# ur-whitelab/hoomd-tf

Measured on AMD Instinct MI355X. Metric: MD steps/sec + achieved HBM GB/s, 131072 particles NN=128 (131k-particle box of the BASELINE metric), higher is better.
Workload: dtype f32

## Files before the change

### hoomd_tf_amd/_lib.py

```python
import ctypes as C
import os

import torch

_HERE = os.path.dirname(os.path.abspath(__file__))
LIB_PATH = os.environ.get("HTF_AMD_LIB") or os.path.join(_HERE, "libhtf_amd.so")

HTF_OK, HTF_ERR_INVALID, HTF_ERR_DEVICE, HTF_ERR_NLIST_OVERFLOW, HTF_ERR_SKEWED_BOX, HTF_ERR_NOMEM = range(6)
HTF_F32, HTF_F64 = 0, 1
HTF_TF2HOOMD, HTF_HOOMD2TF = 0, 1
POT_NONE, POT_LJ, POT_WCA, POT_RINV_POLY, POT_SIMPLE, POT_PAIR_MLP, POT_GAUSS, POT_LJ_PARAM, POT_TOPK_MLP, POT_JIT = range(10)
JIT_READS_OWN_TYPE = 1
OPT_SGD, OPT_ADAM, OPT_NADAM = range(3)
OPT_STATE_FLOATS = 24
ACT_LINEAR, ACT_TANH = 0, 1
MLP_FP32, MLP_BF16, MLP_SPLIT, MLP_SPLIT16 = 0, 1, 2, 3
MAX_POLY_TERMS = 8


class NlistOverflowError(RuntimeError):
    """'Neighbor list is full!' -- tf.errors.InvalidArgumentError upstream
    (simmodel.py:220-224, test_tensorflow.py:830-848)."""


# ... 36 lines not shown
MBOX_MAX_MSG, MBOX_MAX_RANKS, IPC_HANDLE_BYTES = 8, 64, 64


class Mailbox(C.Structure):
    _fields_ = [("remote", C.c_void_p * MBOX_MAX_MSG), ("remote_signal", C.c_void_p * MBOX_MAX_MSG), ("mine", C.c_void_p),
                ("my_signal", C.c_void_p), ("state", C.c_void_p), ("spin_limit", C.c_uint), ("half_units", C.c_uint)]


class ReduceBox(C.Structure):
    _fields_ = [("remote", C.c_void_p * MBOX_MAX_RANKS), ("mine", C.c_void_p), ("state", C.c_void_p), ("spin_limit", C.c_uint),
                ("world", C.c_int), ("rank", C.c_int)]


class Mirror(C.Structure):
    _fields_ = [("src", C.c_void_p * MIRROR_MAX), ("dst", C.c_void_p * MIRROR_MAX), ("words", C.c_uint * MIRROR_MAX), ("n", C.c_uint)]


class Nlist(C.Structure):
    _fields_ = [("box", Box), ("r_list", C.c_double), ("ncell3", C.c_int * 3), ("stencil3", C.c_int * 3), ("pitch", C.c_uint),
                ("type_split", C.c_int)] + [(name, C.c_void_p) for name in (
                    "cell_of", "scratch", "cell_start", "order", "pos_sorted", "ranges", "n_neigh", "head_list", "nlist", "max_neigh",
                    "ref", "counter")] + [("image_L", C.c_double * 3)]


class BrickWork(C.Structure):
    _fields_ = [("key", C.c_void_p), ("order", C.c_void_p), ("sort_scratch", C.c_void_p), ("start1", C.c_void_p),
                ("start2", C.c_void_p), ("tmp_pos", C.c_void_p), ("tmp_vel", C.c_void_p)]


class PotentialDesc(C.Structure):
# ... 279 lines not shown
```

### hoomd_tf_amd/csrc/standin.hip

```cpp
#include <cstdlib>

#include "htf_common.h"
#include "box_math.h"
#include "htf_standin.h"
#include "standin_gate.h"
#include "key_sort.h"

namespace htf {

template <typename T>
__global__ __launch_bounds__(256) void nve_step_kernel(typename Vec4<T>::type *__restrict__ pos,
                                                       typename Vec4<T>::type *__restrict__ vel,
                                                       const typename Vec4<T>::type *__restrict__ force,
                                                       unsigned N, T dt, SBox<T> b) {
    unsigned i = blockIdx.x * blockDim.x + threadIdx.x;
    if (i >= N) return;
    auto p = pos[i];
    auto v = vel[i];
    nve_advance<T>(p, v, force[i], dt, b);
    pos[i] = p;
    vel[i] = v;
}

template <typename T>
__global__ __launch_bounds__(1024) void max_disp_kernel(const typename Vec4<T>::type *__restrict__ pos,
                                                        const typename Vec4<T>::type *__restrict__ ref, unsigned N,
                                                        SBox<T> b, float *__restrict__ out) {
    __shared__ float s_max[16];
    unsigned i = blockIdx.x * blockDim.x + threadIdx.x;
    float d2 = 0.f;
    if (i < N) {
        auto p = pos[i];
        auto r = ref[i];
        T dx = mimg<T>(p.x - r.x, b.L[0], b.Linv[0], b.periodic[0]);
        T dy = mimg<T>(p.y - r.y, b.L[1], b.Linv[1], b.periodic[1]);
        T dz = mimg<T>(p.z - r.z, b.L[2], b.Linv[2], b.periodic[2]);
        d2 = (float)(dx * dx + dy * dy + dz * dz);
        if (!(d2 == d2)) d2 = 0.f;
    }
    for (int m = 1; m < 64; m <<= 1) d2 = fmaxf(d2, __shfl_xor(d2, m));
    if ((threadIdx.x & 63) == 0) s_max[threadIdx.x >> 6] = d2;
    __syncthreads();
    if (threadIdx.x < 16) {
        d2 = s_max[threadIdx.x];
        for (int m = 1; m < 16; m <<= 1) d2 = fmaxf(d2, __shfl_xor(d2, m));
        if (threadIdx.x == 0 && __float_as_uint(d2) > *(volatile unsigned *)out)
            atomicMax((unsigned *)out, __float_as_uint(d2));
    }
}

template <typename T>
__global__ __launch_bounds__(1024) void check_disp_kernel(const typename Vec4<T>::type *__restrict__ pos,
                                                          const typename Vec4<T>::type *__restrict__ ref, unsigned N,
                                                          SBox<T> b, unsigned *__restrict__ work, float *__restrict__ out,
                                                          float *__restrict__ h_out, htfs_mirror mirror) {
    __shared__ float s_max[16];
    __shared__ unsigned s_last;
    unsigned i = blockIdx.x * blockDim.x + threadIdx.x;
    float d2 = 0.f;
    if (i < N) {
        auto p = pos[i];
        auto r = ref[i];
        T dx = mimg<T>(p.x - r.x, b.L[0], b.Linv[0], b.periodic[0]);
        T dy = mimg<T>(p.y - r.y, b.L[1], b.Linv[1], b.periodic[1]);
        T dz = mimg<T>(p.z - r.z, b.L[2], b.Linv[2], b.periodic[2]);
        d2 = (float)(dx * dx + dy * dy + dz * dz);
        if (!(d2 == d2)) d2 = 0.f;
    }
    for (int m = 1; m < 64; m <<= 1) d2 = fmaxf(d2, __shfl_xor(d2, m));
    if ((threadIdx.x & 63) == 0) s_max[threadIdx.x >> 6] = d2;
    if (threadIdx.x == 0) s_last = 0u;
    __syncthreads();
    if (threadIdx.x < 16) {
        d2 = s_max[threadIdx.x];
        for (int m = 1; m < 16; m <<= 1) d2 = fmaxf(d2, __shfl_xor(d2, m));
        if (threadIdx.x == 0) {
            if (__float_as_uint(d2) > *(volatile unsigned *)work) atomicMax(work, __float_as_uint(d2));
            __threadfence();
            if (atomicAdd(work + 1, 1u) == gridDim.x - 1u) s_last = 1u;
        }
    }
    __syncthreads();
    if (s_last == 0u) return;
// ... 4 lines not shown
    }
    __threadfence_system();
    __syncthreads();
    if (threadIdx.x == 0) {
        const float worst = __uint_as_float(atomicExch(work, 0u));
        const unsigned cycle = __float_as_uint(out[1]) + 1u;
        out[0] = worst;
        out[1] = __uint_as_float(cycle);
        work[1] = 0u;
        if (h_out != nullptr) {
            h_out[0] = worst;
            __threadfence_system();
            *(volatile unsigned *)(h_out + 1) = cycle;
        }
    }
}

template <typename T>
__device__ __forceinline__ int cell_coord(T x, T lo, T Linv, int n) {
    int c = (int)floor((x - lo) * Linv * (T)n);
    return c < 0 ? 0 : (c >= n ? n - 1 : c);
}

template <typename T>
__global__ __launch_bounds__(256) void cell_index_kernel(const typename Vec4<T>::type *__restrict__ pos, unsigned Ntot,
                                                         SBox<T> b, int nx, int ny, int nz,
                                                         unsigned *__restrict__ cell_of, Gate gate) {
    if (gate.closed()) return;
    unsigned i = blockIdx.x * blockDim.x + threadIdx.x;
    if (i >= Ntot) return;
// ... 47 lines not shown
        o.x = cell_start[rowbase + a0];
        o.y = (cell_start[rowbase + a1 + 1] - o.x) | (wrap_y << kRangeWrapShift) | (wrap_z << (kRangeWrapShift + 2));
        if (b1 >= b0) {
            o.z = cell_start[rowbase + b0];
            o.w = (cell_start[rowbase + b1 + 1] - o.z) | ((b0 == 0 ? 2u : 1u) << kRangeWrapShift);
        }
    }
    table[t] = o;
}
__global__ __launch_bounds__(256) void cell_ranges_kernel(RangesArgs a, Gate gate) {
    if (gate.closed()) return;
    cell_ranges_body(blockIdx.x * blockDim.x + threadIdx.x, a);
}

template <typename T, int G, bool SHIFT>
__global__ __launch_bounds__(256) void build_nlist_kernel(const typename Vec4<T>::type *__restrict__ pos,
                                                          const typename Vec4<T>::type *__restrict__ pos_sorted,
                                                          unsigned N, SBox<T> b, T rl2, int nx, int ny, int nz,
                                                          int wx, int wy, int wz,
                                                          const unsigned *__restrict__ cell_start, unsigned pitch,
                                                          int type_split,
                                                          unsigned *__restrict__ n_neigh, unsigned *__restrict__ head_list,
                                                          unsigned *__restrict__ nlist, unsigned *__restrict__ max_neigh,
                                                          const uint4 *__restrict__ ranges, Gate gate) {
    if (gate.closed()) return;
    const unsigned lane = threadIdx.x & 63u, g = lane % G, sub = lane / G;
    const unsigned i = ((blockIdx.x * blockDim.x + threadIdx.x) >> 6) * (64 / G) + sub;
    const bool in_range = i < N;
    const auto pi = pos[in_range ? i : 0];
    const bool active = in_range && !is_inert(pi.x);
    const int cx = cell_coord<T>(pi.x, b.lo[0], b.Linv[0], nx);
    const int cy = cell_coord<T>(pi.y, b.lo[1], b.Linv[1], ny);
    const int cz = cell_coord<T>(pi.z, b.lo[2], b.Linv[2], nz);
    const bool side_i = type_split >= 0 && scalar_as_int(pi.w) >= type_split;
    unsigned count = 0;
    unsigned *row = nlist + (size_t)(active ? i : 0) * pitch;
    const int nrow = (2 * wy + 1) * (2 * wz + 1);
    const uint4 *mine = ranges + (size_t)((cz * ny + cy) * nx + cx) * nrow;
    uint4 rg_next = active ? mine[0] : make_uint4(0u, 0u, 0u, 0u);
    for (int r = 0; r < nrow; ++r) {
// ... 25 lines not shown
                unsigned long long hits = ballot64(m_idx < n) & ballot64(k != i) & ballot64(ddx * ddx + ddy * ddy + ddz * ddz <= rl2);
                if (type_split >= 0) {
                    asm volatile("" ::: "memory");
                    hits &= ballot64(((tag & kTagSide) != 0u) == side_i);
                }
                const unsigned seg = (unsigned)(hits >> (G * sub)) & (G >= 32 ? ~0u : ((1u << G) - 1u));
                const unsigned rank = count + (unsigned)__popc(seg & ((1u << g) - 1u));
                if (inverse_ballot64(hits) && rank < pitch) row[rank] = k;
                count += (unsigned)__popc(seg);
            }
        }
    }
    if (in_range && g == 0) {
        n_neigh[i] = count < pitch ? count : pitch;
        head_list[i] = i * pitch;
        if (count > *(volatile unsigned *)max_neigh) atomicMax(max_neigh, count);
    }
}


__device__ __forceinline__ void set_tag(float &w, unsigned tag) { w = __uint_as_float(tag); }
__device__ __forceinline__ void set_tag(double &w, unsigned tag) { w = __longlong_as_double((long long)tag); }
__device__ __forceinline__ float bcast_lane_t(float v, unsigned lane) {
    return __int_as_float(__builtin_amdgcn_readlane(__float_as_int(v), (int)lane));
}
__device__ __forceinline__ double bcast_lane_t(double v, unsigned lane) {
    const long long q = __double_as_longlong(v);
    const unsigned lo = (unsigned)__builtin_amdgcn_readlane((int)(unsigned)q, (int)lane);
    const unsigned hi = (unsigned)__builtin_amdgcn_readlane((int)(unsigned)(q >> 32), (int)lane);
    return __longlong_as_double((long long)(((unsigned long long)hi << 32) | lo));
}
__device__ __forceinline__ unsigned bperm_u(unsigned lane_idx, unsigned v) {
    return (unsigned)__builtin_amdgcn_ds_bpermute((int)(lane_idx << 2), (int)v);
}
__device__ __forceinline__ float bperm_t(unsigned lane_idx, float v) { return __uint_as_float(bperm_u(lane_idx, __float_as_uint(v))); }
__device__ __forceinline__ double bperm_t(unsigned lane_idx, double v) {
    const unsigned long long q = (unsigned long long)__double_as_longlong(v);
    const unsigned lo = bperm_u(lane_idx, (unsigned)q), hi = bperm_u(lane_idx, (unsigned)(q >> 32));
    return __longlong_as_double((long long)(((unsigned long long)hi << 32) | lo));
}
constexpr int kCellBatch = 8;

template <typename T, bool SHIFT>
__global__ __launch_bounds__(256) void build_nlist_cells_kernel(const typename Vec4<T>::type *__restrict__ pos_sorted, unsigned N,
                                                                SBox<T> b, T rl2, unsigned ncell, int nrow,
                                                                const unsigned *__restrict__ cell_start, unsigned pitch,
                                                                int type_split, unsigned *__restrict__ n_neigh,
                                                                unsigned *__restrict__ head_list, unsigned *__restrict__ nlist,
                                                                unsigned *__restrict__ max_neigh,
                                                                const uint4 *__restrict__ ranges, unsigned split, Gate gate) {
    if (gate.closed()) return;
    using V4 = typename Vec4<T>::type;
    const unsigned lane = threadIdx.x & 63u;
    const unsigned wv = __builtin_amdgcn_readfirstlane((blockIdx.x * blockDim.x + threadIdx.x) >> 6);
    const unsigned c = wv / split, b0 = wv % split;
    if (c >= ncell) return;
    const unsigned p_begin = cell_start[c], p_end = cell_start[c + 1];
    if (p_begin + b0 * (unsigned)kCellBatch >= p_end) return;
    if (p_end - p_begin <= 64u) {
        const bool local = lane < p_end - p_begin && ((unsigned)scalar_as_int(pos_sorted[p_begin + lane].w) & ~kTagSide) < N;
        if (ballot64(local) == 0ull) return;
    }

    unsigned beg = 0u, len = 0u;
    T shx = (T)0, shy = (T)0, shz = (T)0;
    if (lane < 2u * (unsigned)nrow) {
// ... 81 lines not shown
                    hits &= ballot64(((tag ^ tag_p[p]) & kTagSide) == 0u);
                }
                const unsigned rank = __builtin_amdgcn_mbcnt_hi((unsigned)(hits >> 32), __builtin_amdgcn_mbcnt_lo((unsigned)hits, count[p]));
                if (inverse_ballot64(hits) && rank < pitch) nlist[row_p[p] + rank] = k;
                count[p] += (unsigned)__builtin_popcountll(hits);
            }
        }
        unsigned cnt = 0u;
#pragma unroll
        for (int p = 0; p < kCellBatch; ++p) cnt = lane == (unsigned)p ? count[p] : cnt;
        if (lane < np) {
            const unsigned i = my_tag & ~kTagSide;
            if (i < N) {
                n_neigh[i] = cnt < pitch ? cnt : pitch;
                head_list[i] = i * pitch;
                if (cnt > *(volatile unsigned *)max_neigh) atomicMax(max_neigh, cnt);
            }
        }
    }
}

}

using namespace htf;

extern "C" int htfs_nve_step(void *d_pos, void *d_vel, const void *d_force, int dtype, unsigned N, double dt,
                             const htf_box *box, htf_stream stream) {
    HTF_REQUIRE(d_pos && d_vel && d_force && box, "htfs_nve_step: null pointer");
    if (N == 0) return HTF_OK;
    unsigned grid = (N + 255) / 256;
    if (dtype == HTF_F32)
        hipLaunchKernelGGL((nve_step_kernel<float>), dim3(grid), dim3(256), 0, (hipStream_t)stream, (float4 *)d_pos, (float4 *)d_vel, (const float4 *)d_force, N, (float)dt, make_sbox<float>(box));
    else
        hipLaunchKernelGGL((nve_step_kernel<double>), dim3(grid), dim3(256), 0, (hipStream_t)stream, (double4 *)d_pos, (double4 *)d_vel, (const double4 *)d_force, N, dt, make_sbox<double>(box));
// ... 30 lines not shown
        hipLaunchKernelGGL((check_disp_kernel<float>), dim3(grid), dim3(1024), 0, (hipStream_t)stream, (const float4 *)d_pos, (const float4 *)d_ref, N, make_sbox<float>(box), d_work, d_out, h_out, mr);
    else
        hipLaunchKernelGGL((check_disp_kernel<double>), dim3(grid), dim3(1024), 0, (hipStream_t)stream, (const double4 *)d_pos, (const double4 *)d_ref, N, make_sbox<double>(box), d_work, d_out, h_out, mr);
    return check_launch("check_disp_kernel");
}

namespace htf {
struct Reimage {
    double L[3], c[3];
};
template <typename T>
__device__ __forceinline__ T reimage1(T x, double L, double c) {
    return L > 0.0 ? (T)((double)x - L * rint(((double)x - c) / L)) : x;
}

template <typename V>
__global__ __launch_bounds__(256) void bins_finish_kernel(RangesArgs ra, unsigned nb_ranges, V *__restrict__ dest, const V *__restrict__ src,
                                                          const int *__restrict__ order, unsigned n, int type_split, V *__restrict__ ref,
                                                          unsigned n_ref, unsigned *__restrict__ counter, Reimage im, Gate gate) {
    if (gate.closed()) return;
    if (blockIdx.x < nb_ranges) {
        cell_ranges_body(blockIdx.x * blockDim.x + threadIdx.x, ra);
        return;
    }
    const unsigned i = (blockIdx.x - nb_ranges) * blockDim.x + threadIdx.x;
    if (i == 0 && counter != nullptr) *counter += 1u;
    if (i >= n || i >= ra.cell_start[ra.nx * ra.ny * ra.nz]) return;
    const unsigned k = (unsigned)order[i];
    V p = src[k];
    if (ref != nullptr && k < n_ref) ref[k] = p;
    p.x = reimage1(p.x, im.L[0], im.c[0]);
    p.y = reimage1(p.y, im.L[1], im.c[1]);
    p.z = reimage1(p.z, im.L[2], im.c[2]);
    set_tag(p.w, k | ((type_split >= 0 && scalar_as_int(p.w) >= type_split) ? kTagSide : 0u));
    dest[i] = p;
}

template <typename T>
__global__ __launch_bounds__(256) void cell_index_count_kernel(const typename Vec4<T>::type *__restrict__ pos, unsigned Ntot, SBox<T> b,
                                                               int nx, int ny, int nz, unsigned *__restrict__ cell_of,
                                                               unsigned *__restrict__ count, Reimage im, Gate gate) {
    if (gate.closed()) return;
    unsigned i = blockIdx.x * blockDim.x + threadIdx.x;
    if (i >= Ntot) return;
    auto p = pos[i];
    if (is_inert(p.x)) {
        cell_of[i] = kDeadCell;
        return;
    }
    int cx = cell_coord<T>(reimage1(p.x, im.L[0], im.c[0]), b.lo[0], b.Linv[0], nx);
// ... 78 lines not shown
}

__global__ __launch_bounds__(256) void cell_scatter_kernel(const unsigned *__restrict__ cell_of, unsigned n,
                                                           unsigned *__restrict__ cursor, unsigned *__restrict__ order, Gate gate) {
    if (gate.closed()) return;
    const unsigned i = blockIdx.x * blockDim.x + threadIdx.x;
    if (i < n && cell_of[i] != kDeadCell) order[atomicAdd(&cursor[cell_of[i]], 1u)] = i;
}

__global__ __launch_bounds__(256) void cell_order_kernel(const unsigned *__restrict__ start, unsigned ncell,
                                                         unsigned *__restrict__ order, unsigned *__restrict__ count, Gate gate) {
    if (gate.closed()) return;
    const unsigned c = blockIdx.x * blockDim.x + threadIdx.x;
    if (c >= ncell) return;
    count[c] = 0u;
    const unsigned b = start[c], e = start[c + 1];
    for (unsigned i = b + 1; i < e; ++i) {
        const unsigned v = order[i];
        unsigned j = i;
        while (j > b && order[j - 1] > v) {
            order[j] = order[j - 1];
            --j;
        }
        order[j] = v;
    }
}
}

static int zero_counts(unsigned *count, unsigned ncell, hipStream_t s) {
    HTF_REQUIRE(((uintptr_t)count & 15) == 0, "binning scratch must be 16-byte aligned (cell_scan_kernel reads it with 16-byte loads)");
    HTF_CHECK_HIP(hipMemsetAsync(count, 0, (size_t)ncell * sizeof(unsigned), s));
    return HTF_OK;
}

extern "C" int htfs_cell_sort(const unsigned *d_cell_of, unsigned Ntot, unsigned ncell, unsigned *d_scratch,
                              unsigned *d_cell_start, unsigned *d_order, htf_stream stream) {
    using namespace htf;
    HTF_REQUIRE(d_cell_of && d_scratch && d_cell_start && d_order, "htfs_cell_sort: null pointer");
    HTF_REQUIRE(ncell > 0, "htfs_cell_sort: no cells");
    hipStream_t s = (hipStream_t)stream;
// ... 120 lines not shown
}

extern "C" int htfs_cell_index(const void *d_pos, int dtype, unsigned Ntot, const htf_box *box, const int *ncell3,
                               unsigned *d_cell_of, htf_stream stream) {
    HTF_REQUIRE(d_pos && box && ncell3 && d_cell_of, "htfs_cell_index: null pointer");
    if (Ntot == 0) return HTF_OK;
    unsigned grid = (Ntot + 255) / 256;
    if (dtype == HTF_F32)
        hipLaunchKernelGGL((cell_index_kernel<float>), dim3(grid), dim3(256), 0, (hipStream_t)stream, (const float4 *)d_pos, Ntot, make_sbox<float>(box), ncell3[0], ncell3[1], ncell3[2], d_cell_of, kOpenGate);
    else
        hipLaunchKernelGGL((cell_index_kernel<double>), dim3(grid), dim3(256), 0, (hipStream_t)stream, (const double4 *)d_pos, Ntot, make_sbox<double>(box), ncell3[0], ncell3[1], ncell3[2], d_cell_of, kOpenGate);
    return check_launch("cell_index_kernel");
}

struct FinishArgs {
    unsigned n;
    htf::Reimage im;
};

static int build_nlist_impl(const htfs_nlist *l, const void *d_pos, int dtype, unsigned N, htf_stream stream, htf::Gate gate,
                            const FinishArgs *fin) {
    using namespace htf;
    HTF_REQUIRE(l && d_pos && l->pos_sorted && l->cell_start && l->n_neigh && l->head_list && l->nlist && l->max_neigh,
                "htfs_build_nlist: null pointer");
    const htf_box *box = &l->box;
    const int *ncell3 = l->ncell3, *stencil3 = l->stencil3;
    const unsigned *d_cell_start = l->cell_start;
    const void *d_pos_sorted = l->pos_sorted;
    const unsigned pitch = l->pitch;
    const int type_split = l->type_split;
    const double r_list = l->r_list;
    unsigned *d_n_neigh = l->n_neigh, *d_head_list = l->head_list, *d_nlist = l->nlist, *d_max_neigh = l->max_neigh;
    HTF_REQUIRE(pitch > 0, "htfs_build_nlist: pitch must be > 0");
    for (int d = 0; d < 3; ++d) {
        const double w = (box->hi[d] - box->lo[d]) / ncell3[d];
        const int sw = stencil3[d];
        HTF_REQUIRE((sw == 0 && ncell3[d] == 1) || (sw >= 1 && sw <= 2 && ncell3[d] >= 2 * sw + 1 && w * sw >= r_list * (1.0 - 1e-12)),
                    "htfs_build_nlist: along %d need 1 cell, or >= 2w+1 cells with w cells spanning r_list (got %d cells of %g, stencil %d, r_list %g)",
                    d, ncell3[d], w, sw, r_list);
    }
    if (N == 0) return HTF_OK;
    const unsigned ncell = (unsigned)(ncell3[0] * ncell3[1] * ncell3[2]);
    const unsigned nrow = (unsigned)((2 * stencil3[1] + 1) * (2 * stencil3[2] + 1));
    HTF_REQUIRE(l->ranges && ((uintptr_t)l->ranges & 15) == 0, "htfs_build_nlist: ranges must be a 16-byte aligned table of 4 * ncell * rows words");
    uint4 *d_ranges = (uint4 *)l->ranges;
    const RangesArgs ra = {ncell3[0], ncell3[1], ncell3[2], stencil3[0], stencil3[1], stencil3[2], (int)box->periodic[0],
                           (int)box->periodic[1], (int)box->periodic[2], d_cell_start, d_ranges, d_max_neigh};
    const unsigned nb_ranges = (ncell * nrow + 255) / 256;
    if (fin == nullptr) {
        hipLaunchKernelGGL(cell_ranges_kernel, dim3(nb_ranges), dim3(256), 0, (hipStream_t)stream, ra, gate);
    } else {
        const unsigned nb = nb_ranges + (fin->n + 255) / 256 + (fin->n == 0 ? 1u : 0u);
        if (dtype == HTF_F32)
            hipLaunchKernelGGL((bins_finish_kernel<float4>), dim3(nb), dim3(256), 0, (hipStream_t)stream, ra, nb_ranges, (float4 *)l->pos_sorted,
                               (const float4 *)d_pos, (const int *)l->order, fin->n, type_split, (float4 *)l->ref, N, l->counter, fin->im, gate);
        else
            hipLaunchKernelGGL((bins_finish_kernel<double4>), dim3(nb), dim3(256), 0, (hipStream_t)stream, ra, nb_ranges, (double4 *)l->pos_sorted,
                               (const double4 *)d_pos, (const int *)l->order, fin->n, type_split, (double4 *)l->ref, N, l->counter, fin->im, gate);
    }
    const bool fine = stencil3[0] == 2 || stencil3[1] == 2 || stencil3[2] == 2;
#define HTFS_NL(T, V4, G)                                                                                              \
    if (shift) HTFS_NL_(T, V4, G, true); else HTFS_NL_(T, V4, G, false)
#define HTFS_NL_(T, V4, G, S)                                                                                          \
    hipLaunchKernelGGL((build_nlist_kernel<T, G, S>), dim3((N + 4 * (64 / G) - 1) / (4 * (64 / G))), dim3(256), 0, (hipStream_t)stream, \
                       (const V4 *)d_pos, (const V4 *)d_pos_sorted, N, make_sbox<T>(box), (T)(r_list * r_list), ncell3[0],  \
                       ncell3[1], ncell3[2], stencil3[0], stencil3[1], stencil3[2], d_cell_start, pitch,      \
                       type_split, d_n_neigh, d_head_list, d_nlist, d_max_neigh, (const uint4 *)d_ranges, gate)
#define HTFS_NLC(T, V4)                                                                                                \
    if (shift) HTFS_NLC_(T, V4, true); else HTFS_NLC_(T, V4, false)
#define HTFS_NLC_(T, V4, S)                                                                                            \
    hipLaunchKernelGGL((build_nlist_cells_kernel<T, S>), dim3((ncell * cell_split + 3) / 4), dim3(256), 0, (hipStream_t)stream, \
                       (const V4 *)d_pos_sorted, N, make_sbox<T>(box), (T)(r_list * r_list), ncell, (int)nrow, d_cell_start, pitch, \
                       type_split, d_n_neigh, d_head_list, d_nlist, d_max_neigh, (const uint4 *)d_ranges, cell_split, gate)
    bool shift = true;
    for (int d = 0; d < 3; ++d) shift = shift && (!box->periodic[d] || ncell3[d] >= 7);
#ifdef HTF_AB_VARIANTS
    static const bool per_particle = std::getenv("HTFS_NLIST_PER_PARTICLE") != nullptr, per_cell = std::getenv("HTFS_NLIST_PER_CELL") != nullptr;
#else
    constexpr bool per_particle = false, per_cell = false;
#endif
    const bool reimaged = fin != nullptr && (fin->im.L[0] > 0.0 || fin->im.L[1] > 0.0 || fin->im.L[2] > 0.0);
    const bool by_cell = per_cell || reimaged || (!per_particle && ncell >= 1024u);
    const unsigned cell_split = ncell <= 12288u ? 2u : 1u;
    if (by_cell) {
        if (dtype == HTF_F32) { HTFS_NLC(float, float4); } else { HTFS_NLC(double, double4); }
    } else if (dtype == HTF_F32) {
        if (fine) { HTFS_NL(float, float4, 8); } else { HTFS_NL(float, float4, 16); }
    } else {
        if (fine) { HTFS_NL(double, double4, 8); } else { HTFS_NL(double, double4, 16); }
    }
#undef HTFS_NL
#undef HTFS_NL_
#undef HTFS_NLC
#undef HTFS_NLC_
    return check_launch("build_nlist_kernel");
}

extern "C" int htfs_build_nlist(const htfs_nlist *nl, const void *d_pos, int dtype, unsigned N, htf_stream stream) {
    return build_nlist_impl(nl, d_pos, dtype, N, stream, htf::kOpenGate, nullptr);
}

static int rebuild_nlist_impl(const htfs_nlist *l, const void *d_pos, int dtype, unsigned N, unsigned Ntot, bool scratch_clean,
                              htf_stream stream, htf::Gate gate) {
    using namespace htf;
    HTF_REQUIRE(l && d_pos && l->cell_of && l->scratch && l->cell_start && l->order && l->pos_sorted, "htfs_rebuild_nlist: null pointer");
    HTF_REQUIRE(Ntot >= N, "htfs_rebuild_nlist: Ntot %u < N %u", Ntot, N);
    if (N == 0) return HTF_OK;
    const htf_box *box = &l->box;
    const int *ncell3 = l->ncell3;
    const unsigned ncell = (unsigned)(ncell3[0] * ncell3[1] * ncell3[2]);
    HTF_REQUIRE(ncell > 0, "htfs_rebuild_nlist: no cells");
    hipStream_t s = (hipStream_t)stream;
    unsigned *count = l->scratch, *cursor = l->scratch + ncell;
    if (!scratch_clean)
        if (int rc = zero_counts(count, ncell, s)) return rc;
    const unsigned grid = (Ntot + 255) / 256;
    Reimage im = {};
    for (int d = 0; d < 3; ++d) {
        im.L[d] = !box->periodic[d] ? l->image_L[d] : 0.0;
        im.c[d] = 0.5 * (box->lo[d] + box->hi[d]);
        HTF_REQUIRE(im.L[d] == 0.0 || im.L[d] >= box->hi[d] - box->lo[d], "htfs_rebuild_nlist: image length %g along axis %d is shorter than the grid", im.L[d], d);
    }
    if (dtype == HTF_F32)
        hipLaunchKernelGGL((cell_index_count_kernel<float>), dim3(grid), dim3(256), 0, s, (const float4 *)d_pos, Ntot, make_sbox<float>(box),
                           ncell3[0], ncell3[1], ncell3[2], l->cell_of, count, im, gate);
    else
        hipLaunchKernelGGL((cell_index_count_kernel<double>), dim3(grid), dim3(256), 0, s, (const double4 *)d_pos, Ntot, make_sbox<double>(box),
                           ncell3[0], ncell3[1], ncell3[2], l->cell_of, count, im, gate);
    hipLaunchKernelGGL(cell_scan_kernel, dim3((ncell + kScanChunk - 1) / kScanChunk), dim3(kScanThreads), 0, s, count, ncell, l->cell_start, cursor, gate);
    hipLaunchKernelGGL(cell_scatter_kernel, dim3(grid), dim3(256), 0, s, l->cell_of, Ntot, cursor, l->order, gate);
    hipLaunchKernelGGL(cell_order_kernel, dim3((ncell + 255) / 256), dim3(256), 0, s, l->cell_start, ncell, l->order, count, gate);
    const FinishArgs fin = {Ntot, im};
    return build_nlist_impl(l, d_pos, dtype, N, stream, gate, &fin);
}

extern "C" int htfs_rebuild_nlist(const htfs_nlist *nl, const void *d_pos, int dtype, unsigned N, unsigned Ntot, int scratch_clean,
                                  htf_stream stream) {
    return rebuild_nlist_impl(nl, d_pos, dtype, N, Ntot, scratch_clean != 0, stream, htf::kOpenGate);
}

extern "C" int htfs_check_rebuild_nlist(const htfs_nlist *nl, const void *d_pos, int dtype, unsigned N, unsigned Ntot, int scratch_clean,
                                        float *d_disp2, double threshold2, unsigned *d_stat2, unsigned *h_stat2, htf_stream stream) {
    HTF_REQUIRE(nl && nl->ref && d_disp2 && d_stat2, "htfs_check_rebuild_nlist: null pointer");
    if (N == 0) return HTF_OK;
    HTF_CHECK_HIP(hipMemsetAsync(d_disp2, 0, sizeof(float), (hipStream_t)stream));
    int rc = htfs_max_displacement2(d_pos, nl->ref, dtype, N, &nl->box, d_disp2, stream);
    if (rc != HTF_OK) return rc;
    htfs_nlist l = *nl;
    l.max_neigh = d_stat2;
    l.counter = d_stat2 + 1;
    rc = rebuild_nlist_impl(&l, d_pos, dtype, N, Ntot, scratch_clean != 0, stream, htf::Gate{d_disp2, (float)threshold2});
    if (rc != HTF_OK) return rc;
    if (h_stat2 != nullptr)
        HTF_CHECK_HIP(hipMemcpyAsync(h_stat2, d_stat2, 2 * sizeof(unsigned), hipMemcpyDeviceToHost, (hipStream_t)stream));
    return HTF_OK;
}
```

### hoomd_tf_amd/standin.py

```python
import ctypes as C
import math
import os

import numpy as np
import torch

from . import _lib, ops
from ._lib import lib, check
from .ops import raw_stream


def fcc_positions(n_cells, rho):
    a = (4.0 / rho) ** (1.0 / 3.0)
    L = n_cells * a
    ijk = np.stack(np.meshgrid(*[np.arange(n_cells)] * 3, indexing="ij"), -1).reshape(-1, 3)
    base = np.array([[0.25, 0.25, 0.25], [0.75, 0.75, 0.25], [0.75, 0.25, 0.75], [0.25, 0.75, 0.75]])
    pos = ((ijk[:, None, :] + base[None]) * a).reshape(-1, 3) - L / 2
    return pos, np.array([L, L, L]), a


def sc_positions(n_cells, rho):
    a = (1.0 / rho) ** (1.0 / 3.0)
    L = n_cells * a
    ijk = np.stack(np.meshgrid(*[np.arange(n_cells)] * 3, indexing="ij"), -1).reshape(-1, 3)
# ... 97 lines not shown
        self.sys = system
        self.deferred_reference = bool(deferred_reference)
        self._rule = None
        self._dd_prev = None
        self._dd_i = 0
        self.device_decision = bool(device_decision)
        self.sort_particles = bool(sort_particles)
        self.r_cut = float(r_cut)
        self.r_buff = float(r_buff)
        self.check_period = int(check_period)
        self._desc = _lib.Nlist()
        self.pitch = pitch
        self.n_neigh = self.head_list = self.nlist = None
        self.type_split = -1
        self._ref = None
        self._disp = torch.zeros(1, dtype=torch.float32, device=system.device)
        self._max = torch.zeros(1, dtype=torch.int32, device=system.device)
        self._desc.max_neigh = self._max.data_ptr()
        self.n_builds = 0
        self._subscribers = []
        self.domain = None
        self._sbox_key = None
        self._scr_n = None
        self._grid = None
        self._scratch_clean = None
        self._step_done = None
        self._capturing = False
        self._stat = self._stat_host = self._stat_event = None
        self._max_host = self._max_event = None
        self._mirrored = False

# ... 758 lines not shown
```

### include/htf_standin.h

```cpp
#ifndef HTF_STANDIN_H_
#define HTF_STANDIN_H_
#include "htf_amd.h"
#ifdef __cplusplus
extern "C" {
#endif

HTF_API int htfs_nve_step(void *d_pos, void *d_vel, const void *d_force, int dtype, unsigned N,
                          double dt, const htf_box *box, htf_stream stream);

HTF_API int htfs_max_displacement2(const void *d_pos, const void *d_ref, int dtype, unsigned N,
                                   const htf_box *box, float *d_out, htf_stream stream);

#define HTFS_MIRROR_MAX 4
typedef struct htfs_mirror {
    const void *src[HTFS_MIRROR_MAX];
    void *dst[HTFS_MIRROR_MAX];
    unsigned words[HTFS_MIRROR_MAX];
    unsigned n;
} htfs_mirror;
HTF_API int htfs_check_displacement2(const void *d_pos, const void *d_ref, int dtype, unsigned N, const htf_box *box,
                                     unsigned *d_work, float *d_out, float *h_out, const htfs_mirror *mirror, htf_stream stream);

#define HTFS_RANGE_WORDS(ncell, stencil_y, stencil_z) (4u * (size_t)(ncell) * (2u * (stencil_y) + 1u) * (2u * (stencil_z) + 1u))
typedef struct htfs_nlist {
// ... 19 lines not shown
} htfs_nlist;

HTF_API int htfs_cell_index(const void *d_pos, int dtype, unsigned Ntot, const htf_box *box,
                            const int *ncell3, unsigned *d_cell_of, htf_stream stream);
HTF_API int htfs_cell_sort(const unsigned *d_cell_of, unsigned Ntot, unsigned ncell, unsigned *d_scratch,
                           unsigned *d_cell_start, unsigned *d_order, htf_stream stream);
HTF_API int htfs_gather4_tagged(void *d_dest, const void *d_src, const int *d_order, int dtype, unsigned n, int type_split,
                                htf_stream stream);
HTF_API int htfs_gather4_tagged_live(void *d_dest, const void *d_src, const int *d_order, int dtype, unsigned n_max,
                                     const unsigned *d_n_live, int type_split, htf_stream stream);
HTF_API int htfs_build_nlist(const htfs_nlist *nl, const void *d_pos, int dtype, unsigned N, htf_stream stream);

HTF_API int htfs_rebuild_nlist(const htfs_nlist *nl, const void *d_pos, int dtype, unsigned N, unsigned Ntot, int scratch_clean,
                               htf_stream stream);

HTF_API int htfs_check_rebuild_nlist(const htfs_nlist *nl, const void *d_pos, int dtype, unsigned N, unsigned Ntot, int scratch_clean,
                                     float *d_disp2, double threshold2, unsigned *d_stat2, unsigned *h_stat2, htf_stream stream);

HTF_API int htfs_slab_classify(const void *d_pos, int dtype, unsigned N, const void *d_bounds, int world, int rank,
                               double r_ghost, unsigned *d_key, htf_stream stream);

HTF_API int htfs_key_sort16(const unsigned *d_key, unsigned N, unsigned *d_scratch, unsigned *d_start, unsigned *d_order,
                            htf_stream stream);

#define HTFS_MAX_SEGMENTS 16
HTF_API int htfs_segment_copy(void *d_dst, const void *d_src, unsigned row_bytes, unsigned n_segments,
                              const unsigned *src_start, const unsigned *dst_start, const unsigned *count, htf_stream stream);

#define HTFS_BRICK_MAX_MSG 8
#define HTFS_BRICK_MAX_P 64
// ... 126 lines not shown
```

Before: 13410.

## Fuse displacement check and stat reporting into nlist rebuild kernels

Replaces the memset plus max-displacement launch with a single self-resetting check_gate kernel that publishes the max displacement via a ticket counter. The separate cell_order sort kernel is folded into bins_finish, which now runs per cell and sorts small cells in registers with an odd-even network. The host memcpy of the stat words is replaced by a last-workgroup tree ticket inside the nlist build kernel that writes the stats directly to host memory. Together these remove several launches and a copy per step, at the cost of extra atomics and a per-cell finish whose load balance depends on cell occupancy.

```diff
diff --git a/hoomd_tf_amd/_lib.py b/hoomd_tf_amd/_lib.py
--- a/hoomd_tf_amd/_lib.py
+++ b/hoomd_tf_amd/_lib.py
@@ -74,6 +74,9 @@
 
 class Mirror(C.Structure):
     _fields_ = [("src", C.c_void_p * MIRROR_MAX), ("dst", C.c_void_p * MIRROR_MAX), ("words", C.c_uint * MIRROR_MAX), ("n", C.c_uint)]
+
+
+HTFS_CHECK_WORDS = 2112
 
 
 class Nlist(C.Structure):
diff --git a/hoomd_tf_amd/csrc/standin.hip b/hoomd_tf_amd/csrc/standin.hip
--- a/hoomd_tf_amd/csrc/standin.hip
+++ b/hoomd_tf_amd/csrc/standin.hip
@@ -22,6 +22,15 @@
     vel[i] = v;
 }
 
+template <typename T, typename V4>
+__device__ __forceinline__ float row_disp2(const V4 &p, const V4 &r, const SBox<T> &b) {
+    T dx = mimg<T>(p.x - r.x, b.L[0], b.Linv[0], b.periodic[0]);
+    T dy = mimg<T>(p.y - r.y, b.L[1], b.Linv[1], b.periodic[1]);
+    T dz = mimg<T>(p.z - r.z, b.L[2], b.Linv[2], b.periodic[2]);
+    float d2 = (float)(dx * dx + dy * dy + dz * dz);
+    return d2 == d2 ? d2 : 0.f;
+}
+
 template <typename T>
 __global__ __launch_bounds__(1024) void max_disp_kernel(const typename Vec4<T>::type *__restrict__ pos,
                                                         const typename Vec4<T>::type *__restrict__ ref, unsigned N,
@@ -29,15 +38,7 @@
     __shared__ float s_max[16];
     unsigned i = blockIdx.x * blockDim.x + threadIdx.x;
     float d2 = 0.f;
-    if (i < N) {
-        auto p = pos[i];
-        auto r = ref[i];
-        T dx = mimg<T>(p.x - r.x, b.L[0], b.Linv[0], b.periodic[0]);
-        T dy = mimg<T>(p.y - r.y, b.L[1], b.Linv[1], b.periodic[1]);
-        T dz = mimg<T>(p.z - r.z, b.L[2], b.Linv[2], b.periodic[2]);
-        d2 = (float)(dx * dx + dy * dy + dz * dz);
-        if (!(d2 == d2)) d2 = 0.f;
-    }
+    if (i < N) d2 = row_disp2<T>(pos[i], ref[i], b);
     for (int m = 1; m < 64; m <<= 1) d2 = fmaxf(d2, __shfl_xor(d2, m));
     if ((threadIdx.x & 63) == 0) s_max[threadIdx.x >> 6] = d2;
     __syncthreads();
@@ -58,15 +59,7 @@
     __shared__ unsigned s_last;
     unsigned i = blockIdx.x * blockDim.x + threadIdx.x;
     float d2 = 0.f;
-    if (i < N) {
-        auto p = pos[i];
-        auto r = ref[i];
-        T dx = mimg<T>(p.x - r.x, b.L[0], b.Linv[0], b.periodic[0]);
-        T dy = mimg<T>(p.y - r.y, b.L[1], b.Linv[1], b.periodic[1]);
-        T dz = mimg<T>(p.z - r.z, b.L[2], b.Linv[2], b.periodic[2]);
-        d2 = (float)(dx * dx + dy * dy + dz * dz);
-        if (!(d2 == d2)) d2 = 0.f;
-    }
+    if (i < N) d2 = row_disp2<T>(pos[i], ref[i], b);
     for (int m = 1; m < 64; m <<= 1) d2 = fmaxf(d2, __shfl_xor(d2, m));
     if ((threadIdx.x & 63) == 0) s_max[threadIdx.x >> 6] = d2;
     if (threadIdx.x == 0) s_last = 0u;
@@ -101,6 +94,68 @@
             *(volatile unsigned *)(h_out + 1) = cycle;
         }
     }
+}
+
+constexpr unsigned kCheckDisp = 0;
+constexpr unsigned kCheckWork = 1;
+constexpr unsigned kCheckTicket = 2;
+constexpr unsigned kSearchRoot = 32;
+constexpr unsigned kSearchLeaf0 = 64;
+constexpr unsigned kTicketLeaves = 64, kTicketStride = 32;
+static_assert(kSearchLeaf0 + kTicketLeaves * kTicketStride == HTFS_CHECK_WORDS, "htf_standin.h HTFS_CHECK_WORDS");
+
+__device__ __forceinline__ void atomic_max_performed(unsigned *word, unsigned v) {
+    const unsigned old = atomicMax(word, v);
+    asm volatile("" ::"v"(old) : "memory");
+}
+__device__ __forceinline__ unsigned atomic_read(unsigned *word) { return __hip_atomic_load(word, __ATOMIC_RELAXED, __HIP_MEMORY_SCOPE_AGENT); }
+__device__ __forceinline__ void atomic_write(unsigned *word, unsigned v) { __hip_atomic_store(word, v, __ATOMIC_RELAXED, __HIP_MEMORY_SCOPE_AGENT); }
+
+template <typename T>
+__global__ __launch_bounds__(1024) void check_gate_kernel(const typename Vec4<T>::type *__restrict__ pos,
+                                                          const typename Vec4<T>::type *__restrict__ ref, unsigned N,
+                                                          SBox<T> b, unsigned *__restrict__ words) {
+    __shared__ float s_max[16];
+    unsigned i = blockIdx.x * blockDim.x + threadIdx.x;
+    float d2 = 0.f;
+    if (i < N) d2 = row_disp2<T>(pos[i], ref[i], b);
+    for (int m = 1; m < 64; m <<= 1) d2 = fmaxf(d2, __shfl_xor(d2, m));
+    if ((threadIdx.x & 63) == 0) s_max[threadIdx.x >> 6] = d2;
+    __syncthreads();
+    if (threadIdx.x >= 16) return;
+    d2 = s_max[threadIdx.x];
+    for (int m = 1; m < 16; m <<= 1) d2 = fmaxf(d2, __shfl_xor(d2, m));
+    if (threadIdx.x != 0) return;
+    if (__float_as_uint(d2) > atomic_read(words + kCheckWork)) atomic_max_performed(words + kCheckWork, __float_as_uint(d2));
+    if (atomicAdd(words + kCheckTicket, 1u) != gridDim.x - 1u) return;
+    words[kCheckDisp] = atomicExch(words + kCheckWork, 0u);
+    atomic_write(words + kCheckTicket, 0u);
+}
+
+__device__ __forceinline__ bool last_workgroup(unsigned *words) {
+    const unsigned nb = gridDim.x, leaf = blockIdx.x % kTicketLeaves;
+    const unsigned in_leaf = (nb - leaf + kTicketLeaves - 1u) / kTicketLeaves, leaves = nb < kTicketLeaves ? nb : kTicketLeaves;
+    unsigned *lw = words + kSearchLeaf0 + leaf * kTicketStride;
+    if (atomicAdd(lw, 1u) != in_leaf - 1u) return false;
+    atomic_write(lw, 0u);
+    if (atomicAdd(words + kSearchRoot, 1u) != leaves - 1u) return false;
+    atomic_write(words + kSearchRoot, 0u);
+    return true;
+}
+
+struct StatOut {
+    unsigned *tickets;
+    unsigned *d_stat2, *h_stat2;
+};
+__device__ __forceinline__ void report_stat(const StatOut &so) {
+    if (so.tickets == nullptr) return;
+    __syncthreads();
+    if (threadIdx.x != 0 || !last_workgroup(so.tickets)) return;
+    __hip_atomic_store(so.h_stat2, atomicMax(so.d_stat2, 0u), __ATOMIC_RELAXED, __HIP_MEMORY_SCOPE_SYSTEM);
+    __hip_atomic_store(so.h_stat2 + 1, so.d_stat2[1], __ATOMIC_RELAXED, __HIP_MEMORY_SCOPE_SYSTEM);
+}
+__device__ __forceinline__ void row_count_max(unsigned *max_neigh, unsigned cnt) {
+    if (cnt > *(volatile unsigned *)max_neigh) atomic_max_performed(max_neigh, cnt);
 }
 
 template <typename T>
@@ -178,16 +233,15 @@
 }
 
 template <typename T, int G, bool SHIFT>
-__global__ __launch_bounds__(256) void build_nlist_kernel(const typename Vec4<T>::type *__restrict__ pos,
-                                                          const typename Vec4<T>::type *__restrict__ pos_sorted,
-                                                          unsigned N, SBox<T> b, T rl2, int nx, int ny, int nz,
-                                                          int wx, int wy, int wz,
-                                                          const unsigned *__restrict__ cell_start, unsigned pitch,
-                                                          int type_split,
-                                                          unsigned *__restrict__ n_neigh, unsigned *__restrict__ head_list,
-                                                          unsigned *__restrict__ nlist, unsigned *__restrict__ max_neigh,
-                                                          const uint4 *__restrict__ ranges, Gate gate) {
-    if (gate.closed()) return;
+__device__ __forceinline__ void build_nlist_body(const typename Vec4<T>::type *__restrict__ pos,
+                                                 const typename Vec4<T>::type *__restrict__ pos_sorted,
+                                                 unsigned N, const SBox<T> &b, T rl2, int nx, int ny, int nz,
+                                                 int wx, int wy, int wz,
+                                                 const unsigned *__restrict__ cell_start, unsigned pitch,
+                                                 int type_split,
+                                                 unsigned *__restrict__ n_neigh, unsigned *__restrict__ head_list,
+                                                 unsigned *__restrict__ nlist, unsigned *__restrict__ max_neigh,
+                                                 const uint4 *__restrict__ ranges) {
     const unsigned lane = threadIdx.x & 63u, g = lane % G, sub = lane / G;
     const unsigned i = ((blockIdx.x * blockDim.x + threadIdx.x) >> 6) * (64 / G) + sub;
     const bool in_range = i < N;
@@ -243,8 +297,23 @@
     if (in_range && g == 0) {
         n_neigh[i] = count < pitch ? count : pitch;
         head_list[i] = i * pitch;
-        if (count > *(volatile unsigned *)max_neigh) atomicMax(max_neigh, count);
-    }
+        row_count_max(max_neigh, count);
+    }
+}
+template <typename T, int G, bool SHIFT>
+__global__ __launch_bounds__(256) void build_nlist_kernel(const typename Vec4<T>::type *__restrict__ pos,
+                                                          const typename Vec4<T>::type *__restrict__ pos_sorted,
+                                                          unsigned N, SBox<T> b, T rl2, int nx, int ny, int nz,
+                                                          int wx, int wy, int wz,
+                                                          const unsigned *__restrict__ cell_start, unsigned pitch,
+                                                          int type_split,
+                                                          unsigned *__restrict__ n_neigh, unsigned *__restrict__ head_list,
+                                                          unsigned *__restrict__ nlist, unsigned *__restrict__ max_neigh,
+                                                          const uint4 *__restrict__ ranges, Gate gate, StatOut so) {
+    if (gate.closed()) return;
+    build_nlist_body<T, G, SHIFT>(pos, pos_sorted, N, b, rl2, nx, ny, nz, wx, wy, wz, cell_start, pitch, type_split, n_neigh, head_list,
+                                  nlist, max_neigh, ranges);
+    report_stat(so);
 }
 
 
@@ -271,14 +340,13 @@
 constexpr int kCellBatch = 8;
 
 template <typename T, bool SHIFT>
-__global__ __launch_bounds__(256) void build_nlist_cells_kernel(const typename Vec4<T>::type *__restrict__ pos_sorted, unsigned N,
-                                                                SBox<T> b, T rl2, unsigned ncell, int nrow,
-                                                                const unsigned *__restrict__ cell_start, unsigned pitch,
-                                                                int type_split, unsigned *__restrict__ n_neigh,
-                                                                unsigned *__restrict__ head_list, unsigned *__restrict__ nlist,
-                                                                unsigned *__restrict__ max_neigh,
-                                                                const uint4 *__restrict__ ranges, unsigned split, Gate gate) {
-    if (gate.closed()) return;
+__device__ __forceinline__ void build_nlist_cells_body(const typename Vec4<T>::type *__restrict__ pos_sorted, unsigned N,
+                                                       const SBox<T> &b, T rl2, unsigned ncell, int nrow,
+                                                       const unsigned *__restrict__ cell_start, unsigned pitch,
+                                                       int type_split, unsigned *__restrict__ n_neigh,
+                                                       unsigned *__restrict__ head_list, unsigned *__restrict__ nlist,
+                                                       unsigned *__restrict__ max_neigh,
+                                                       const uint4 *__restrict__ ranges, unsigned split) {
     using V4 = typename Vec4<T>::type;
     const unsigned lane = threadIdx.x & 63u;
     const unsigned wv = __builtin_amdgcn_readfirstlane((blockIdx.x * blockDim.x + threadIdx.x) >> 6);
@@ -390,10 +458,23 @@
             if (i < N) {
                 n_neigh[i] = cnt < pitch ? cnt : pitch;
                 head_list[i] = i * pitch;
-                if (cnt > *(volatile unsigned *)max_neigh) atomicMax(max_neigh, cnt);
+                row_count_max(max_neigh, cnt);
             }
         }
     }
+}
+template <typename T, bool SHIFT>
+__global__ __launch_bounds__(256) void build_nlist_cells_kernel(const typename Vec4<T>::type *__restrict__ pos_sorted, unsigned N,
+                                                                SBox<T> b, T rl2, unsigned ncell, int nrow,
+                                                                const unsigned *__restrict__ cell_start, unsigned pitch,
+                                                                int type_split, unsigned *__restrict__ n_neigh,
+                                                                unsigned *__restrict__ head_list, unsigned *__restrict__ nlist,
+                                                                unsigned *__restrict__ max_neigh,
+                                                                const uint4 *__restrict__ ranges, unsigned split, Gate gate, StatOut so) {
+    if (gate.closed()) return;
+    build_nlist_cells_body<T, SHIFT>(pos_sorted, N, b, rl2, ncell, nrow, cell_start, pitch, type_split, n_neigh, head_list, nlist,
+                                     max_neigh, ranges, split);
+    report_stat(so);
 }
 
 }
@@ -454,26 +535,75 @@
     return L > 0.0 ? (T)((double)x - L * rint(((double)x - c) / L)) : x;
 }
 
+__device__ __forceinline__ void sort_cell_in_place(unsigned *__restrict__ order, unsigned b, unsigned e) {
+    for (unsigned i = b + 1; i < e; ++i) {
+        const unsigned v = order[i];
+        unsigned j = i;
+        while (j > b && order[j - 1] > v) {
+            order[j] = order[j - 1];
+            --j;
+        }
+        order[j] = v;
+    }
+}
+
 template <typename V>
-__global__ __launch_bounds__(256) void bins_finish_kernel(RangesArgs ra, unsigned nb_ranges, V *__restrict__ dest, const V *__restrict__ src,
-                                                          const int *__restrict__ order, unsigned n, int type_split, V *__restrict__ ref,
-                                                          unsigned n_ref, unsigned *__restrict__ counter, Reimage im, Gate gate) {
-    if (gate.closed()) return;
-    if (blockIdx.x < nb_ranges) {
-        cell_ranges_body(blockIdx.x * blockDim.x + threadIdx.x, ra);
-        return;
-    }
-    const unsigned i = (blockIdx.x - nb_ranges) * blockDim.x + threadIdx.x;
-    if (i == 0 && counter != nullptr) *counter += 1u;
-    if (i >= n || i >= ra.cell_start[ra.nx * ra.ny * ra.nz]) return;
-    const unsigned k = (unsigned)order[i];
-    V p = src[k];
+__device__ __forceinline__ void finish_row(V p, unsigned k, unsigned i, V *__restrict__ dest, V *__restrict__ ref, unsigned n_ref,
+                                           int type_split, const Reimage &im) {
     if (ref != nullptr && k < n_ref) ref[k] = p;
     p.x = reimage1(p.x, im.L[0], im.c[0]);
     p.y = reimage1(p.y, im.L[1], im.c[1]);
     p.z = reimage1(p.z, im.L[2], im.c[2]);
     set_tag(p.w, k | ((type_split >= 0 && scalar_as_int(p.w) >= type_split) ? kTagSide : 0u));
     dest[i] = p;
+}
+
+constexpr int kCellReg = 8;
+template <typename V>
+__global__ __launch_bounds__(256) void bins_finish_kernel(RangesArgs ra, unsigned nb_ranges, V *__restrict__ dest, const V *__restrict__ src,
+                                                          unsigned *__restrict__ order, unsigned *__restrict__ count, int type_split,
+                                                          V *__restrict__ ref, unsigned n_ref, unsigned *__restrict__ counter, Reimage im,
+                                                          Gate gate) {
+    if (gate.closed()) return;
+    if (blockIdx.x < nb_ranges) {
+        cell_ranges_body(blockIdx.x * blockDim.x + threadIdx.x, ra);
+        return;
+    }
+    const unsigned c = (blockIdx.x - nb_ranges) * blockDim.x + threadIdx.x;
+    if (c == 0 && counter != nullptr) *counter += 1u;
+    if (c >= (unsigned)(ra.nx * ra.ny * ra.nz)) return;
+    const unsigned b = ra.cell_start[c], m = ra.cell_start[c + 1] - b;
+    count[c] = 0u;
+    if (m <= (unsigned)kCellReg) {
+        unsigned k[kCellReg];
+#pragma unroll
+        for (int j = 0; j < kCellReg; ++j) k[j] = (unsigned)j < m ? order[b + j] : ~0u;
+#pragma unroll
+        for (int r = 0; r < kCellReg; ++r)
+#pragma unroll
+            for (int j = r & 1; j + 1 < kCellReg; j += 2) {
+                const unsigned lo = min(k[j], k[j + 1]), hi = max(k[j], k[j + 1]);
+                k[j] = lo;
+                k[j + 1] = hi;
+            }
+        V p[kCellReg];
+#pragma unroll
+        for (int j = 0; j < kCellReg; ++j)
+            if ((unsigned)j < m) {
+                order[b + j] = k[j];
+                p[j] = src[k[j]];
+            }
+#pragma unroll
+        for (int j = 0; j < kCellReg; ++j)
+            if ((unsigned)j < m) finish_row(p[j], k[j], b + j, dest, ref, n_ref, type_split, im);
+    } else {
+        sort_cell_in_place(order, b, b + m);
+#pragma unroll 4
+        for (unsigned i = b; i < b + m; ++i) {
+            const unsigned k = order[i];
+            finish_row(src[k], k, i, dest, ref, n_ref, type_split, im);
+        }
+    }
 }
 
 template <typename T>
@@ -582,16 +712,7 @@
     const unsigned c = blockIdx.x * blockDim.x + threadIdx.x;
     if (c >= ncell) return;
     count[c] = 0u;
-    const unsigned b = start[c], e = start[c + 1];
-    for (unsigned i = b + 1; i < e; ++i) {
-        const unsigned v = order[i];
-        unsigned j = i;
-        while (j > b && order[j - 1] > v) {
-            order[j] = order[j - 1];
-            --j;
-        }
-        order[j] = v;
-    }
+    sort_cell_in_place(order, start[c], start[c + 1]);
 }
 }
 
@@ -742,12 +863,11 @@
 }
 
 struct FinishArgs {
-    unsigned n;
     htf::Reimage im;
 };
 
 static int build_nlist_impl(const htfs_nlist *l, const void *d_pos, int dtype, unsigned N, htf_stream stream, htf::Gate gate,
-                            const FinishArgs *fin) {
+                            const FinishArgs *fin, const htf::StatOut &so) {
     using namespace htf;
     HTF_REQUIRE(l && d_pos && l->pos_sorted && l->cell_start && l->n_neigh && l->head_list && l->nlist && l->max_neigh,
                 "htfs_build_nlist: null pointer");
@@ -778,13 +898,13 @@
     if (fin == nullptr) {
         hipLaunchKernelGGL(cell_ranges_kernel, dim3(nb_ranges), dim3(256), 0, (hipStream_t)stream, ra, gate);
     } else {
-        const unsigned nb = nb_ranges + (fin->n + 255) / 256 + (fin->n == 0 ? 1u : 0u);
+        const unsigned nb = nb_ranges + (ncell + 255) / 256;
         if (dtype == HTF_F32)
             hipLaunchKernelGGL((bins_finish_kernel<float4>), dim3(nb), dim3(256), 0, (hipStream_t)stream, ra, nb_ranges, (float4 *)l->pos_sorted,
-                               (const float4 *)d_pos, (const int *)l->order, fin->n, type_split, (float4 *)l->ref, N, l->counter, fin->im, gate);
+                               (const float4 *)d_pos, l->order, l->scratch, type_split, (float4 *)l->ref, N, l->counter, fin->im, gate);
         else
             hipLaunchKernelGGL((bins_finish_kernel<double4>), dim3(nb), dim3(256), 0, (hipStream_t)stream, ra, nb_ranges, (double4 *)l->pos_sorted,
-                               (const double4 *)d_pos, (const int *)l->order, fin->n, type_split, (double4 *)l->ref, N, l->counter, fin->im, gate);
+                               (const double4 *)d_pos, l->order, l->scratch, type_split, (double4 *)l->ref, N, l->counter, fin->im, gate);
     }
     const bool fine = stencil3[0] == 2 || stencil3[1] == 2 || stencil3[2] == 2;
 #define HTFS_NL(T, V4, G)                                                                                              \
@@ -793,13 +913,13 @@
     hipLaunchKernelGGL((build_nlist_kernel<T, G, S>), dim3((N + 4 * (64 / G) - 1) / (4 * (64 / G))), dim3(256), 0, (hipStream_t)stream, \
                        (const V4 *)d_pos, (const V4 *)d_pos_sorted, N, make_sbox<T>(box), (T)(r_list * r_list), ncell3[0],  \
                        ncell3[1], ncell3[2], stencil3[0], stencil3[1], stencil3[2], d_cell_start, pitch,      \
-                       type_split, d_n_neigh, d_head_list, d_nlist, d_max_neigh, (const uint4 *)d_ranges, gate)
+                       type_split, d_n_neigh, d_head_list, d_nlist, d_max_neigh, (const uint4 *)d_ranges, gate, so)
 #define HTFS_NLC(T, V4)                                                                                                \
     if (shift) HTFS_NLC_(T, V4, true); else HTFS_NLC_(T, V4, false)
 #define HTFS_NLC_(T, V4, S)                                                                                            \
     hipLaunchKernelGGL((build_nlist_cells_kernel<T, S>), dim3((ncell * cell_split + 3) / 4), dim3(256), 0, (hipStream_t)stream, \
                        (const V4 *)d_pos_sorted, N, make_sbox<T>(box), (T)(r_list * r_list), ncell, (int)nrow, d_cell_start, pitch, \
-                       type_split, d_n_neigh, d_head_list, d_nlist, d_max_neigh, (const uint4 *)d_ranges, cell_split, gate)
+                       type_split, d_n_neigh, d_head_list, d_nlist, d_max_neigh, (const uint4 *)d_ranges, cell_split, gate, so)
     bool shift = true;
     for (int d = 0; d < 3; ++d) shift = shift && (!box->periodic[d] || ncell3[d] >= 7);
 #ifdef HTF_AB_VARIANTS
@@ -825,11 +945,11 @@
 }
 
 extern "C" int htfs_build_nlist(const htfs_nlist *nl, const void *d_pos, int dtype, unsigned N, htf_stream stream) {
-    return build_nlist_impl(nl, d_pos, dtype, N, stream, htf::kOpenGate, nullptr);
+    return build_nlist_impl(nl, d_pos, dtype, N, stream, htf::kOpenGate, nullptr, htf::StatOut{});
 }
 
 static int rebuild_nlist_impl(const htfs_nlist *l, const void *d_pos, int dtype, unsigned N, unsigned Ntot, bool scratch_clean,
-                              htf_stream stream, htf::Gate gate) {
+                              htf_stream stream, htf::Gate gate, const htf::StatOut &so) {
     using namespace htf;
     HTF_REQUIRE(l && d_pos && l->cell_of && l->scratch && l->cell_start && l->order && l->pos_sorted, "htfs_rebuild_nlist: null pointer");
     HTF_REQUIRE(Ntot >= N, "htfs_rebuild_nlist: Ntot %u < N %u", Ntot, N);
@@ -857,29 +977,29 @@
                            ncell3[0], ncell3[1], ncell3[2], l->cell_of, count, im, gate);
     hipLaunchKernelGGL(cell_scan_kernel, dim3((ncell + kScanChunk - 1) / kScanChunk), dim3(kScanThreads), 0, s, count, ncell, l->cell_start, cursor, gate);
     hipLaunchKernelGGL(cell_scatter_kernel, dim3(grid), dim3(256), 0, s, l->cell_of, Ntot, cursor, l->order, gate);
-    hipLaunchKernelGGL(cell_order_kernel, dim3((ncell + 255) / 256), dim3(256), 0, s, l->cell_start, ncell, l->order, count, gate);
-    const FinishArgs fin = {Ntot, im};
-    return build_nlist_impl(l, d_pos, dtype, N, stream, gate, &fin);
+    const FinishArgs fin = {im};
+    return build_nlist_impl(l, d_pos, dtype, N, stream, gate, &fin, so);
 }
 
 extern "C" int htfs_rebuild_nlist(const htfs_nlist *nl, const void *d_pos, int dtype, unsigned N, unsigned Ntot, int scratch_clean,
                                   htf_stream stream) {
-    return rebuild_nlist_impl(nl, d_pos, dtype, N, Ntot, scratch_clean != 0, stream, htf::kOpenGate);
+    return rebuild_nlist_impl(nl, d_pos, dtype, N, Ntot, scratch_clean != 0, stream, htf::kOpenGate, htf::StatOut{});
 }
 
 extern "C" int htfs_check_rebuild_nlist(const htfs_nlist *nl, const void *d_pos, int dtype, unsigned N, unsigned Ntot, int scratch_clean,
                                         float *d_disp2, double threshold2, unsigned *d_stat2, unsigned *h_stat2, htf_stream stream) {
-    HTF_REQUIRE(nl && nl->ref && d_disp2 && d_stat2, "htfs_check_rebuild_nlist: null pointer");
+    HTF_REQUIRE(nl && nl->ref && d_pos && d_disp2 && d_stat2, "htfs_check_rebuild_nlist: null pointer");
     if (N == 0) return HTF_OK;
-    HTF_CHECK_HIP(hipMemsetAsync(d_disp2, 0, sizeof(float), (hipStream_t)stream));
-    int rc = htfs_max_displacement2(d_pos, nl->ref, dtype, N, &nl->box, d_disp2, stream);
-    if (rc != HTF_OK) return rc;
+    unsigned *words = (unsigned *)d_disp2;
+    const unsigned grid = (N + 1023) / 1024;
+    if (dtype == HTF_F32)
+        hipLaunchKernelGGL((check_gate_kernel<float>), dim3(grid), dim3(1024), 0, (hipStream_t)stream, (const float4 *)d_pos, (const float4 *)nl->ref, N, make_sbox<float>(&nl->box), words);
+    else
+        hipLaunchKernelGGL((check_gate_kernel<double>), dim3(grid), dim3(1024), 0, (hipStream_t)stream, (const double4 *)d_pos, (const double4 *)nl->ref, N, make_sbox<double>(&nl->box), words);
+    if (int rc = check_launch("check_gate_kernel")) return rc;
     htfs_nlist l = *nl;
     l.max_neigh = d_stat2;
     l.counter = d_stat2 + 1;
-    rc = rebuild_nlist_impl(&l, d_pos, dtype, N, Ntot, scratch_clean != 0, stream, htf::Gate{d_disp2, (float)threshold2});
-    if (rc != HTF_OK) return rc;
-    if (h_stat2 != nullptr)
-        HTF_CHECK_HIP(hipMemcpyAsync(h_stat2, d_stat2, 2 * sizeof(unsigned), hipMemcpyDeviceToHost, (hipStream_t)stream));
-    return HTF_OK;
-}
+    const StatOut so = {h_stat2 != nullptr ? words : nullptr, d_stat2, h_stat2};
+    return rebuild_nlist_impl(&l, d_pos, dtype, N, Ntot, scratch_clean != 0, stream, htf::Gate{d_disp2, (float)threshold2}, so);
+}
diff --git a/hoomd_tf_amd/standin.py b/hoomd_tf_amd/standin.py
--- a/hoomd_tf_amd/standin.py
+++ b/hoomd_tf_amd/standin.py
@@ -135,7 +135,8 @@
         self.n_neigh = self.head_list = self.nlist = None
         self.type_split = -1
         self._ref = None
-        self._disp = torch.zeros(1, dtype=torch.float32, device=system.device)
+        self._check_words = torch.zeros(_lib.HTFS_CHECK_WORDS, dtype=torch.float32, device=system.device)
+        self._disp = self._check_words[:1]
         self._max = torch.zeros(1, dtype=torch.int32, device=system.device)
         self._desc.max_neigh = self._max.data_ptr()
         self.n_builds = 0
diff --git a/include/htf_standin.h b/include/htf_standin.h
--- a/include/htf_standin.h
+++ b/include/htf_standin.h
@@ -57,6 +57,7 @@
 HTF_API int htfs_rebuild_nlist(const htfs_nlist *nl, const void *d_pos, int dtype, unsigned N, unsigned Ntot, int scratch_clean,
                                htf_stream stream);
 
+#define HTFS_CHECK_WORDS 2112
 HTF_API int htfs_check_rebuild_nlist(const htfs_nlist *nl, const void *d_pos, int dtype, unsigned N, unsigned Ntot, int scratch_clean,
                                      float *d_disp2, double threshold2, unsigned *d_stat2, unsigned *h_stat2, htf_stream stream);
 
```

New measurement: 13480, median of 4. No clear change (+0.5%).
